# CliMA/LandHydrology.jl

Measured on AMD Instinct MI355X. Metric: column-cell updates/sec (RHS evals), higher is better.
Workload: dtype f64

## Files before the change

landhydrology.jl_amd/csrc/lh_column_ops.hpp:

```cpp
#pragma once
#include "lh_closures.hpp"

namespace lh {

template <typename M>
__device__ __forceinline__ MathTables stage_math_tables(const double* gtab, double* lds) {
    MathTables t;
    t.log_tab = lds;
    t.exp_tab = lds + 2 * LOG_TAB_N;
    if (M::uses_tables) {
        for (int i = threadIdx.x; i < MATH_TAB_DOUBLES; i += blockDim.x) lds[i] = gtab[i];
        __syncthreads();
    }
    return t;
}

template <typename M>
constexpr int implicit_threads() {
    return M::uses_tables ? 512 : 256;
}
template <typename M>
__device__ __forceinline__ M implicit_math(const double* math_tab) {
    __shared__ double s_tab[M::uses_tables ? MATH_TAB_DOUBLES : 2];
    return M(stage_math_tables<M>(math_tab, s_tab));
}
__device__ __forceinline__ int64_t implicit_lane_column() { return int64_t(blockIdx.x) * blockDim.x + threadIdx.x; }

template <typename FT> struct Bits;
template <> struct Bits<double> { using type = unsigned long long; };
template <> struct Bits<float> { using type = unsigned int; };

__device__ __forceinline__ double fmax_ft(double a, double b) { return __builtin_fmax(a, b); }
__device__ __forceinline__ float fmax_ft(float a, float b) { return __builtin_fmaxf(a, b); }
__device__ __forceinline__ double fmin_ft(double a, double b) { return __builtin_fmin(a, b); }
__device__ __forceinline__ float fmin_ft(float a, float b) { return __builtin_fminf(a, b); }

__device__ __forceinline__ float max_nonneg(float a, float b) {
    return __builtin_bit_cast(float, __builtin_elementwise_max(__builtin_bit_cast(int, a), __builtin_bit_cast(int, b)));
}

__device__ __forceinline__ unsigned xcd_block(int xcd_remap) {
    unsigned blk = blockIdx.x;
    if (xcd_remap) {
        const unsigned per = gridDim.x >> 3;
        if (blk < (per << 3)) blk = (blk & 7u) * per + (blk >> 3);
    }
    return blk;
}

template <typename FT>
__device__ __forceinline__ void set_stage_boundary_values(DevParams<FT>& P, const FT* b) {
    P.bc_value[FACE_BOTTOM][COMP_ENERGY] = b[0];
    P.bc_value[FACE_BOTTOM][COMP_HYDROLOGY] = b[1];
    P.bc_value[FACE_TOP][COMP_ENERGY] = b[2];
    P.bc_value[FACE_TOP][COMP_HYDROLOGY] = b[3];
}

template <typename FT, typename M>
__device__ __forceinline__ void flux_scales(const DevParams<FT>& P, const ColC<FT>& c, FT& Ksc, FT& cgw) {
    Ksc = M::is_production ? c.Ksat : FT(1);
    cgw = M::is_production ? c.cgw : P.cg2;
}

template <typename FT, typename M, int MODEL, bool FACTORS, bool NOICE, bool WANT_DT>
__device__ __forceinline__ void cell_closures(const M& mm, const DevParams<FT>& P, const ColC<FT>& c, FT vl, FT ti,
                                              FT re, FT Ta, bool vgf, FT& T, FT& kap, FT& K, FT& psi, FT& E,
                                              float& dpsi, float& ircs) {
    constexpr bool WATER = (MODEL != MODEL_HEAT), HEAT = (MODEL != MODEL_RICHARDS);
    FT rcs = FT(1);
    T = Ta;
    kap = FT(0);
    K = psi = E = FT(0);
    dpsi = ircs = 0.0f;
    if (HEAT) {
        T = temperature_closure<FT, M, NOICE>(mm, P, c, vl, ti, re, rcs);
        kap = kappa_closure<FT, M, NOICE>(mm, P, c, vl, ti);
// ... 62 lines not shown
```

landhydrology.jl_amd/csrc/lh_kernels_impl.hpp:

```cpp
#pragma once
#include "lh_closures.hpp"
#include "lh_column_ops.hpp"
#include "lh_launch.hpp"
#include "lh_dispatch.hpp"
#include "lh_atmos.hpp"
#include <type_traits>

namespace lh {

template <typename FT, int MODEL, bool FACTORS, bool PERCOL, typename M, int MODE>
constexpr bool f32_coupled_vgpr_constants() {
    if (MODEL != MODEL_COUPLED || PERCOL || !M::is_production || !(MODE == 0 || MODE == 4)) return false;
    if (sizeof(FT) == 4 && MODE == 4) return true;
    return !FACTORS;
}

template <typename FT, int MODEL, bool FACTORS, bool PERCOL, typename M, bool NOICE>
constexpr bool heat_vgpr_constants() {
    return sizeof(FT) == 8 && MODEL != MODEL_RICHARDS && M::is_production && !NOICE;
}

template <typename FT, int MODEL, bool FACTORS, bool PERCOL, typename M, int PF, int MODE, bool NOICE = false>
constexpr int rhs_waves_per_simd() {
    constexpr bool F64 = sizeof(FT) == 8, RICHARDS = MODEL == MODEL_RICHARDS;
// ... 45 lines not shown
template <int CPL_, int PF_, bool NT_, bool SEG_>
struct KCfg {
    static constexpr int CPL = CPL_, PF = PF_;
    static constexpr bool NT = NT_, SEG = SEG_;
};

__device__ __forceinline__ void wave_sync() {
    __builtin_amdgcn_fence(__ATOMIC_RELEASE, "wavefront");
    __builtin_amdgcn_wave_barrier();
    __builtin_amdgcn_fence(__ATOMIC_ACQUIRE, "wavefront");
}

template <typename FT>
__device__ __forceinline__ bool finite(FT x) {
    return x - x == FT(0);
}

template <typename M>
constexpr bool noice_exists(bool factors) { return M::is_production && !factors; }
template <typename M, int MODEL>
constexpr bool robust_vg_exists() { return M::uses_tables && MODEL != MODEL_HEAT; }
template <typename CFG>
constexpr bool robust_shape_exists() { return !CFG::NT && !CFG::SEG; }
template <typename M, int MODE>
constexpr bool rhs_mode_exists() { return M::is_production || MODE == 0; }
template <typename FT, int MODEL, bool FACTORS, bool PERCOL, typename CFG, typename M, int MODE, bool NOICE = false, bool VGF = true>
__global__ void __launch_bounds__((rhs_max_threads<M, rhs_waves_per_simd<FT, MODEL, FACTORS, PERCOL, M, CFG::PF, MODE, NOICE>()>()),
                                  (rhs_min_waves<M, rhs_waves_per_simd<FT, MODEL, FACTORS, PERCOL, M, CFG::PF, MODE, NOICE>()>()))
rhs_kernel(const DevParams<FT> P0, const Planes<FT> IN, const Planes<FT> AUX, const Planes<FT> BASE,
           const Planes<FT> OUT, const FT dt_value, const FT* __restrict__ dt_device) {
    constexpr bool WATER = (MODEL != MODEL_HEAT);
    constexpr bool HEAT = (MODEL != MODEL_RICHARDS);
    constexpr bool TEND_MODE = (MODE == 0 || MODE == 4);
    DevParams<FT> P = P0;
    if constexpr (heat_vgpr_constants<FT, MODEL, FACTORS, PERCOL, M, NOICE>() && TEND_MODE && (!FACTORS || PERCOL || MODE == 4)) {
        auto vr = [](FT& x) { asm volatile("" : "+v"(x)); };
        vr(P.rho_c_ds); vr(P.rhocp_l); vr(P.rhocp_i); vr(P.T_ref); vr(P.kappa_sat_unfrozen);
        vr(P.l2_kappa_sat_unfrozen); vr(P.l2_kappa_sat_frozen); vr(P.kersten_exp_unfrozen);
        vr(P.kersten_exp_frozen); vr(P.neg_b_log2e_sc);
        if (MODE != 4) {
            vr(P.rho_i); vr(P.LH_f0); vr(P.inv_dz); vr(P.half_inv_dz);
            if (FACTORS) { vr(P.gamma); vr(P.T_ref_visc); vr(P.Omega); }
        }
    }
    if constexpr (heat_vgpr_constants<FT, MODEL, FACTORS, PERCOL, M, NOICE>() && MODE == 0 && FACTORS && !PERCOL) {
        auto vr = [](FT& x) { asm volatile("" : "+v"(x)); };
        vr(P.rho_c_ds); vr(P.rhocp_l); vr(P.T_ref);
    }
    constexpr int CPL = CFG::CPL, PF = CFG::PF;
    constexpr bool NT = CFG::NT;
    constexpr bool TEND = (MODE == 0 || MODE == 4);
    constexpr bool WANT_DT = (MODE == 4);
    const FT dt = (!TEND && dt_device) ? *dt_device : dt_value;
    __shared__ double s_tab[M::uses_tables ? MATH_TAB_DOUBLES : 2];
    extern __shared__ __align__(16) unsigned char s_dyn[];
    const int n = P.nlev;
    float* s_red = reinterpret_cast<float*>(s_dyn);
    if (WANT_DT) s_red[threadIdx.x] = 0.0f;
    __shared__ unsigned s_waves_done;
    if (WANT_DT && threadIdx.x == 0) s_waves_done = 0u;
    constexpr bool MAY_PROF = (MODEL == MODEL_HEAT) || (MODEL == MODEL_RICHARDS && FACTORS);
    FT* s_pf = reinterpret_cast<FT*>(s_dyn + (WANT_DT ? ((size_t(blockDim.x) * sizeof(float) + 15) & ~size_t(15)) : 0));
    const FT* pf_T = (MAY_PROF && MODEL == MODEL_RICHARDS) ? P.aux_prof[3] : nullptr;
    const FT* pf_vl = (MAY_PROF && MODEL == MODEL_HEAT) ? P.aux_prof[0] : nullptr;
    const FT* pf_ti = (MAY_PROF && MODEL == MODEL_HEAT) ? P.aux_prof[1] : nullptr;
    if constexpr (MAY_PROF) {
        for (int i = threadIdx.x; i < n; i += blockDim.x) {
            if (pf_T) s_pf[i] = pf_T[i];
            if (pf_vl) s_pf[i] = pf_vl[i];
            if (pf_ti) s_pf[n + i] = pf_ti[i];
        }
    }
    const M mm(stage_math_tables<M>(P.math_tab, s_tab));
    if (!M::uses_tables) __syncthreads();

    unsigned blk = blockIdx.x;
    if (P.xcd_remap) {
        const unsigned per = gridDim.x >> 3;
        if (blk < (per << 3)) blk = (blk & 7u) * per + (blk >> 3);
    }
    const int64_t col0 = (int64_t(blk) * blockDim.x + threadIdx.x) * CPL;
    if (col0 >= P.ncols) return;
    const int64_t stride = P.stride;
    constexpr bool SEG = CFG::SEG;
    const int i_lo = SEG ? int(blockIdx.y) * P.seg_len : 0;
    const int i_hi = SEG ? (i_lo + P.seg_len < n ? i_lo + P.seg_len : n) : n;
    const int i_first = (SEG && i_lo > 0) ? i_lo - 1 : 0;
    const int i_end = (SEG && i_hi < n) ? i_hi + 1 : n;
    const unsigned lane_byte = (unsigned)col0 * (unsigned)sizeof(FT);
    const unsigned row_bytes = (unsigned)(stride * (int64_t)sizeof(FT));
    auto rload = [&](const FT* row, FT (&out)[CPL]) { bload<FT, CPL, NT>(row, row_bytes, lane_byte, out); };
    auto rstore = [&](FT* row, const FT (&in)[CPL]) { bstore<FT, CPL, NT>(row, row_bytes, lane_byte, in); };

    const int64_t in0 = SEG ? stride * i_first : 0, out0 = SEG ? stride * i_lo : 0;
    constexpr bool FROM_K1 = (MODE == 5);
    const FT* r_vl = (MODEL == MODEL_HEAT ? AUX.v[0] : (FROM_K1 ? BASE.v[0] : IN.v[0])) + in0;
    const FT* r_ti = NOICE ? nullptr : (MODEL == MODEL_HEAT ? AUX.v[1] : (TEND ? IN.v[1] : BASE.v[1])) + in0;
    const FT* r_re = HEAT ? (FROM_K1 ? BASE.v[2] : IN.v[2]) + in0 : nullptr;
    const FT* r_k1v = (FROM_K1 && WATER) ? IN.v[0] + in0 : nullptr;
    const FT* r_k1e = (FROM_K1 && HEAT) ? IN.v[2] + in0 : nullptr;
    const bool need_Taux = (MODEL == MODEL_RICHARDS) && FACTORS && P.viscosity_kind;
    const FT* r_Ta = need_Taux ? AUX.v[3] + in0 : nullptr;
    const FT* b_vl = ((MODE == 2 || MODE == 3) && WATER) ? BASE.v[0] + out0 : nullptr;
    const FT* b_re = ((MODE == 2 || MODE == 3) && HEAT) ? BASE.v[2] + out0 : nullptr;
    FT* o_vl = WATER ? OUT.v[0] + out0 : nullptr;
    FT* o_re = HEAT ? OUT.v[2] + out0 : nullptr;

    ColC<FT> c[CPL];
    int64_t colj[CPL];
#pragma unroll
    for (int j = 0; j < CPL; ++j) {
        colj[j] = col0 + j < P.ncols ? col0 + j : P.ncols - 1;
        c[j] = make_colc<FT, M>(P, colj[j], PERCOL);
        if (WATER && !NOICE) finish_colc<FT, M>(mm, c[j]);
        if constexpr (M::uses_tables && WATER && !PERCOL && !HEAT) asm volatile("" : "+v"(c[j].e_log2_alpha));
    }
    if constexpr (f32_coupled_vgpr_constants<FT, MODEL, FACTORS, PERCOL, M, MODE>()) {
        auto vr = [](FT& x) { asm volatile("" : "+v"(x)); };
        ColC<FT>& q = c[0];
        vr(q.nu); vr(q.theta_lim); vr(q.theta_r); vr(q.inv_por); vr(q.e_inv_m); vr(q.e_m); vr(q.e_one);
        vr(q.e_inv_n); vr(q.e_log2_alpha); vr(q.Ksat); vr(q.inv_S_s); vr(q.inv_nu); vr(q.k_dry);
        if (!NOICE) vr(q.l2_por);
#pragma unroll
        for (int j = 1; j < CPL; ++j) c[j] = c[0];
    }

    constexpr bool vgf = VGF && M::uses_tables;
    const FT cgT = P.cg2;
    FT cgw[CPL], Ksc[CPL];
#pragma unroll
    for (int j = 0; j < CPL; ++j) flux_scales<FT, M>(P, c[j], Ksc[j], cgw[j]);

    FT vl[CPL], ti[CPL], re[CPL], Ta[CPL];
    FT vl_n[PF][CPL], ti_n[PF][CPL], re_n[PF][CPL], Ta_n[PF][CPL];
    FT kv_n[PF][CPL], ke_n[PF][CPL];
    FT vl_p[CPL], re_p[CPL];
    FT yv[CPL], ye[CPL], yv_p[CPL], ye_p[CPL];
    FT K_p[CPL], psi_p[CPL], T_p[CPL], kap_p[CPL], E_p[CPL];
    FT Fw_lo[CPL], Fe_lo[CPL];
    FT nf_acc = FT(0);
    float dpsi_p[CPL], ircs_p[CPL], DmaxW[CPL], DmaxT[CPL];
    float DmaxWb[CPL];

#pragma unroll
    for (int j = 0; j < CPL; ++j) {
        K_p[j] = psi_p[j] = T_p[j] = kap_p[j] = E_p[j] = Fw_lo[j] = Fe_lo[j] = FT(0);
        vl_p[j] = re_p[j] = FT(0);
        yv[j] = ye[j] = yv_p[j] = ye_p[j] = FT(0);
        vl[j] = ti[j] = re[j] = FT(0);
        Ta[j] = FT(288);
        dpsi_p[j] = DmaxW[j] = DmaxWb[j] = DmaxT[j] = ircs_p[j] = 0.0f;
    }
    int lev_f = i_first;
    auto fetch = [&](int slot) {
        if (MAY_PROF && pf_vl) {
#pragma unroll
            for (int j = 0; j < CPL; ++j) vl_n[slot][j] = s_pf[lev_f];
        } else rload(r_vl, vl_n[slot]);
        if (!NOICE) {
            if (MAY_PROF && pf_ti) {
#pragma unroll
                for (int j = 0; j < CPL; ++j) ti_n[slot][j] = s_pf[n + lev_f];
            } else rload(r_ti, ti_n[slot]);
        }
        if (HEAT) rload(r_re, re_n[slot]);
        if (need_Taux) {
            if (MAY_PROF && pf_T) {
#pragma unroll
                for (int j = 0; j < CPL; ++j) Ta_n[slot][j] = s_pf[lev_f];
            } else rload(r_Ta, Ta_n[slot]);
        }
        ++lev_f;
        if (FROM_K1 && WATER) { rload(r_k1v, kv_n[slot]); r_k1v += stride; }
        if (FROM_K1 && HEAT) { rload(r_k1e, ke_n[slot]); r_k1e += stride; }
        r_vl += stride;
        if (!NOICE) r_ti += stride;
        if (HEAT) r_re += stride;
        if (need_Taux) r_Ta += stride;
    };
#pragma unroll
    for (int k = 0; k < PF; ++k) {
#pragma unroll
        for (int j = 0; j < CPL; ++j) {
            vl_n[k][j] = ti_n[k][j] = re_n[k][j] = kv_n[k][j] = ke_n[k][j] = FT(0);
            Ta_n[k][j] = FT(288);
        }
        if (i_first + k < i_end) fetch(k);
    }

    auto emit = [&](const FT (&Fw_hi)[CPL], const FT (&Fe_hi)[CPL], const FT (&u_vl)[CPL],
                    const FT (&u_re)[CPL], const FT (&y_vl)[CPL], const FT (&y_re)[CPL]) {
        FT dvl[CPL], dre[CPL];
#pragma unroll
        for (int j = 0; j < CPL; ++j) {
            dvl[j] = WATER ? Fw_lo[j] - Fw_hi[j] : FT(0);
            dre[j] = HEAT ? Fe_lo[j] - Fe_hi[j] : FT(0);
            if (CPL == 1 || col0 + j < P.ncols) {
                if (WATER) nf_acc = fma_ft(dvl[j], FT(0), nf_acc);
                if (HEAT) nf_acc = fma_ft(dre[j], FT(0), nf_acc);
            }
        }
        if (TEND) {
            if (WATER) rstore(o_vl, dvl);
            if (HEAT) rstore(o_re, dre);
        } else {
            auto stage = [&](const FT* brow, FT* orow, const FT (&u)[CPL], const FT (&k)[CPL], const FT (&yb)[CPL]) {
                constexpr int STAGE = MODE == 1 ? 0 : (MODE == 3 ? 2 : 1);
                FT b[CPL] = {}, r[CPL];
                if (MODE == 2 || MODE == 3) rload(brow, b);
#pragma unroll
                for (int j = 0; j < CPL; ++j) {
                    if (FROM_K1) b[j] = yb[j];
                    r[j] = ssprk33_stage_value<FT>(STAGE, b[j], u[j], k[j], dt);
                }
                rstore(orow, r);
            };
            if (WATER) stage(b_vl, o_vl, u_vl, dvl, y_vl);
            if (HEAT) stage(b_re, o_re, u_re, dre, y_re);
        }
        if (WATER) {
            o_vl += stride;
            if (MODE == 2 || MODE == 3) b_vl += stride;
        }
        if (HEAT) {
            o_re += stride;
            if (MODE == 2 || MODE == 3) b_re += stride;
        }
    };

    for (int i0 = i_first; i0 < i_end; i0 += PF) {
#pragma unroll
      for (int k = 0; k < PF; ++k) {
        const int i = i0 + k;
        if (PF > 1 && i >= i_end) break;
#pragma unroll
        for (int j = 0; j < CPL; ++j) {
            vl[j] = vl_n[k][j];
            ti[j] = NOICE ? FT(0) : ti_n[k][j];
            re[j] = re_n[k][j];
            Ta[j] = Ta_n[k][j];
// ... 98 lines not shown
                    DmaxT[j] = max_nonneg(DmaxT[j], 4.0f * float(fmax_ft(kap_f, kap_f > FT(0) ? kap_p[j] : FT(0))) * ircs_p[j]);
                }
            }
        }
        emit(Fw, Fe, vl_p, re_p, yv_p, ye_p);
    }
    if (nf_acc != nf_acc) atomicOr(P.status, 1u);
    if (WANT_DT) {
        float dmax = 0.0f;
#pragma unroll
        for (int j = 0; j < CPL; ++j) {
            const float Dj = max_nonneg(max_nonneg(DmaxW[j] * float(Ksc[j]), DmaxWb[j]) * float(FT(1) / (c[j].n * c[j].m)), DmaxT[j]);
            if ((CPL == 1 || col0 + j < P.ncols) && Dj == Dj) dmax = max_nonneg(dmax, Dj);
        }
        float* seg = s_red + (threadIdx.x & ~63u);
        const unsigned l = threadIdx.x & 63u;
        seg[l] = dmax;
#pragma unroll
        for (unsigned off = 32; off > 0; off >>= 1) {
            wave_sync();
            if (l < off) {
                dmax = max_nonneg(dmax, seg[l + off]);
                seg[l] = dmax;
            }
        }
        if (l == 0) {
            const int64_t first_lane = int64_t(blk) * blockDim.x;
            const int64_t lanes_left = (P.ncols + CPL - 1) / CPL - first_lane;
            const unsigned nwaves = blockDim.x >> 6;
            const unsigned nw = lanes_left >= int64_t(blockDim.x) ? nwaves : unsigned((lanes_left + 63) >> 6);
            if (atomicAdd(&s_waves_done, 1u) == nw - 1u) {
                for (unsigned w = 0; w < nwaves; ++w) dmax = max_nonneg(dmax, s_red[w << 6]);
                if (dmax > 0.0f) bound_publish<FT>(P, dt, dmax);
            }
        }
    }
}

constexpr int CS_FACE_WORDS = 8;
template <int MODEL> constexpr int cs_flux_arrays() {
    return MODEL == MODEL_COUPLED ? 2 : 1;
}
static inline int cs_fetch_tiles(int model, bool noice, bool need_Taux) {
    if (model == MODEL_RICHARDS) return 1 + (noice ? 0 : 1) + (need_Taux ? 2 : 0);
    return 3;
}

template <typename FT, int MODEL, bool FACTORS, bool PERCOL, typename M, bool NOICE = false, bool VGF = true>
__global__ void __launch_bounds__(1024)
column_stepper_kernel(const DevParams<FT> P0, const Planes<FT> Y, const Planes<FT> AUX, const FT dt_value,
                      const FT* __restrict__ dt_device, const int64_t nsteps, const FT* __restrict__ bcv) {
    constexpr bool WATER = (MODEL != MODEL_HEAT);
    constexpr bool HEAT = (MODEL != MODEL_RICHARDS);
    __shared__ double s_tab[M::uses_tables ? MATH_TAB_DOUBLES : 2];
    extern __shared__ __align__(16) unsigned char s_dyn[];
    const int n = P0.nlev;
    const int tpc = (n + 63) & ~63;
    const int slot = int(threadIdx.x) / tpc;
    const int cpb = int(blockDim.x) / tpc;
    const FT dt = dt_device ? *dt_device : dt_value;
    constexpr int NARR = cs_exchange_arrays<MODEL>();
    const StepperLds<FT, MODEL> ex(reinterpret_cast<FT*>(s_dyn) + size_t(slot) * NARR * n, n);
    const M mm(stage_math_tables<M>(P0.math_tab, s_tab));
    if (!M::uses_tables) __syncthreads();
    DevParams<FT> P = P0;
    const int i = int(threadIdx.x) - slot * tpc;
    const unsigned blk = xcd_block(P.xcd_remap);
    const int64_t col_raw = int64_t(blk) * cpb + slot;
    const bool cell = i < n && col_raw < P.ncols;
    const int ic = i < n ? i : n - 1;
    const int64_t col = col_raw < P.ncols ? col_raw : P.ncols - 1;
    ColC<FT> c = make_colc<FT, M>(P, col, PERCOL);
    if (WATER && !NOICE) finish_colc<FT, M>(mm, c);
    constexpr bool vgf = VGF && M::uses_tables;
    const FT cgT = P.cg2;
    FT Ksc, cgw;
    flux_scales<FT, M>(P, c, Ksc, cgw);
    const bool need_Taux = (MODEL == MODEL_RICHARDS) && FACTORS && P.viscosity_kind;
    FT* tiles = reinterpret_cast<FT*>(s_dyn);
    const int64_t col_first = int64_t(blk) * cpb;
    const int tile_n = n * cpb;
    auto request = [&](const FT* plane, int k) {
        for (int e = threadIdx.x; e < tile_n; e += blockDim.x) {
            const int lev = e / cpb, cs = e - lev * cpb;
            if (col_first + cs < P.ncols) tiles[k * tile_n + cs * n + lev] = plane[int64_t(lev) * P.stride + col_first + cs];
        }
    };
    auto fetched = [&](int k) -> FT { return (col_raw < P.ncols) ? tiles[k * tile_n + slot * n + ic] : FT(0); };
    const FT* pf_vl = MODEL == MODEL_HEAT ? P.aux_prof[0] : nullptr;
    const FT* pf_ti = MODEL == MODEL_HEAT ? P.aux_prof[1] : nullptr;
    const FT* pf_T = need_Taux ? P.aux_prof[3] : nullptr;
    if (!pf_vl) request(MODEL == MODEL_HEAT ? AUX.v[0] : Y.v[0], 0);
    if (!NOICE && !pf_ti) request(MODEL == MODEL_HEAT ? AUX.v[1] : Y.v[1], 1);
    if (HEAT) request(Y.v[2], 2);
    if (need_Taux && !pf_T) request(AUX.v[3], 3);
    __syncthreads();
    FT y_vl = pf_vl ? pf_vl[ic] : fetched(0);
    const FT ti = NOICE ? FT(0) : (pf_ti ? pf_ti[ic] : fetched(1));
    FT y_re = HEAT ? fetched(2) : FT(0);
    const FT Ta = need_Taux ? (pf_T ? pf_T[ic] : fetched(3)) : FT(288);
    __syncthreads();
    FT nf_acc = FT(0);
    for (int64_t s = 0; s < nsteps; ++s) {
        FT u_vl = y_vl, u_re = y_re;
#pragma unroll 1
        for (int stage = 0; stage < 3; ++stage) {
            if (bcv) set_stage_boundary_values(P, bcv + (s * 3 + stage) * 4);
// ... 41 lines not shown
            const FT dre = HEAT ? Fe_lo - Fe_hi : FT(0);
            if (cell) {
                if (WATER) nf_acc = fma_ft(dvl, FT(0), nf_acc);
                if (HEAT) nf_acc = fma_ft(dre, FT(0), nf_acc);
            }
            if (WATER) u_vl = ssprk33_stage_value<FT>(stage, y_vl, u_vl, dvl, dt);
            if (HEAT) u_re = ssprk33_stage_value<FT>(stage, y_re, u_re, dre, dt);
            __syncthreads();
        }
        y_vl = u_vl;
        y_re = u_re;
    }
    __syncthreads();
    if (i < n) {
        if (WATER) tiles[slot * n + i] = y_vl;
        if (HEAT) tiles[tile_n + slot * n + i] = y_re;
    }
    __syncthreads();
    for (int e = threadIdx.x; e < tile_n; e += blockDim.x) {
        const int lev = e / cpb, cs = e - lev * cpb;
        if (col_first + cs < P.ncols) {
            const int64_t g = int64_t(lev) * P.stride + col_first + cs;
            if (WATER) Y.v[0][g] = tiles[cs * n + lev];
            if (HEAT) Y.v[2][g] = tiles[tile_n + cs * n + lev];
        }
    }
    if (cell && nf_acc != nf_acc) atomicOr(P.status, 1u);
}

template <typename T>
__device__ __forceinline__ T wave_uniform(const T& x) {
    static_assert(sizeof(T) % 4 == 0, "32-bit words");
    uint32_t w[sizeof(T) / 4];
    __builtin_memcpy(w, &x, sizeof(T));
#pragma unroll
    for (size_t k = 0; k < sizeof(T) / 4; ++k) w[k] = __builtin_amdgcn_readfirstlane(w[k]);
    T r;
    __builtin_memcpy(&r, w, sizeof(T));
    return r;
}

template <typename FT, int MODEL, bool FACTORS, bool PERCOL, typename M, int CW, bool NOICE>
constexpr int cs_wave_min_waves() {
    if (!M::uses_tables || MODEL != MODEL_RICHARDS) return 4;
    if (CW == 1) return 6;
    return (NOICE && !FACTORS) ? 6 : 4;
}
template <typename FT, int MODEL, bool FACTORS, bool PERCOL, typename M, int CW, bool NOICE = false, bool VGF = true, bool BOUND = false>
__global__ void __launch_bounds__(1024, (cs_wave_min_waves<FT, MODEL, FACTORS, PERCOL, M, CW, NOICE>()))
column_stepper_wave_kernel(const DevParams<FT> P0, const Planes<FT> Y, const Planes<FT> AUX, const FT dt_value,
                           const FT* __restrict__ dt_device, const int64_t nsteps, const FT* __restrict__ bcv) {
    constexpr bool WATER = (MODEL != MODEL_HEAT);
    constexpr bool HEAT = (MODEL != MODEL_RICHARDS);
    __shared__ double s_tab[M::uses_tables ? MATH_TAB_DOUBLES : 2];
    extern __shared__ __align__(16) unsigned char s_dyn[];
    const int n = P0.nlev;
    const int slot = int(threadIdx.x) >> 6;
    const int l = int(threadIdx.x) & 63;
    const int cpb = int(blockDim.x) >> 6;
    const FT dt = dt_device ? *dt_device : dt_value;
    constexpr int NEX = cs_exchange_arrays<MODEL>();
    constexpr int NARR = NEX + cs_flux_arrays<MODEL>();
    constexpr size_t COLW = size_t(NARR) * 64 + CS_FACE_WORDS;
    const StepperLds<FT, MODEL> ex(reinterpret_cast<FT*>(s_dyn) + size_t(slot) * COLW, 64);
    FT* sFw = ex.K + size_t(NEX) * 64;
    FT* sFe = WATER ? sFw + 64 : sFw;
    FT* sFace = ex.K + size_t(NARR) * 64;
    const M mm(stage_math_tables<M>(P0.math_tab, s_tab));
    if (!M::uses_tables) __syncthreads();
    DevParams<FT> P = P0;
    const unsigned blk = xcd_block(P.xcd_remap);
    const int64_t col_raw = int64_t(blk) * cpb + slot;
    const int64_t col = col_raw < P.ncols ? col_raw : P.ncols - 1;
    ColC<FT> c = make_colc<FT, M>(P, col, PERCOL);
    if (WATER && !NOICE) finish_colc<FT, M>(mm, c);
    if constexpr (PERCOL) c = wave_uniform(c);
    constexpr bool vgf = VGF && M::uses_tables;
    const FT cgT = P.cg2;
    FT Ksc, cgw;
    flux_scales<FT, M>(P, c, Ksc, cgw);
    const bool need_Taux = (MODEL == MODEL_RICHARDS) && FACTORS && P.viscosity_kind;
    FT* tiles = reinterpret_cast<FT*>(s_dyn);
    const int64_t col_first = int64_t(blk) * cpb;
    const int tile_n = n * cpb;
    auto request = [&](const FT* plane, int k) {
        for (int e = threadIdx.x; e < tile_n; e += blockDim.x) {
            const int lev = e / cpb, cs = e - lev * cpb;
            if (col_first + cs < P.ncols) tiles[k * tile_n + cs * n + lev] = plane[int64_t(lev) * P.stride + col_first + cs];
        }
    };
    const FT* pf_vl = MODEL == MODEL_HEAT ? P.aux_prof[0] : nullptr;
    const FT* pf_ti = MODEL == MODEL_HEAT ? P.aux_prof[1] : nullptr;
    const FT* pf_T = need_Taux ? P.aux_prof[3] : nullptr;
    if (!pf_vl) request(MODEL == MODEL_HEAT ? AUX.v[0] : Y.v[0], 0);
    if (!NOICE && !pf_ti) request(MODEL == MODEL_HEAT ? AUX.v[1] : Y.v[1], 1);
    if (HEAT) request(Y.v[2], 2);
    if (need_Taux && !pf_T) request(AUX.v[3], 3);
    __syncthreads();
    FT y_vl[CW], y_re[CW], ti[CW], Ta[CW];
    bool act[CW];
#pragma unroll
    for (int q = 0; q < CW; ++q) {
        const int i = CW * l + q;
        const int ic = i < n ? i : n - 1;
        act[q] = i < n && col_raw < P.ncols;
        const bool have = col_raw < P.ncols;
        y_vl[q] = pf_vl ? pf_vl[ic] : (have ? tiles[slot * n + ic] : FT(0));
// ... 183 lines not shown
            } else {
                const FaceState<FT> fs = face_state<FT, M, MODEL, FACTORS, NOICE>(mm, P, c, face, col, bv, bti, bT, vgf);
                K_f = fs.K;
                kap_f = fs.kap;
            }
            const FT K_c = bK * Ksc;
            DmaxW = max_nonneg(DmaxW, 2.0f * float(bK) * bdpsi);
            DmaxWb = max_nonneg(DmaxWb, 4.0f * float(fmax_ft(K_f, K_f > FT(0) ? K_c : FT(0))) * bdpsi);
            if (HEAT) {
                DmaxT = max_nonneg(DmaxT, 2.0f * float(bkap) * bircs);
                DmaxT = max_nonneg(DmaxT, 4.0f * float(fmax_ft(kap_f, kap_f > FT(0) ? bkap : FT(0))) * bircs);
            }
        };
        if (at_bottom || at_top) boundary_terms(at_bottom ? FACE_BOTTOM : FACE_TOP, at_bottom ? hoist_b : hoist_t, at_bottom ? 0 : qt);
        if (at_bottom && at_top) boundary_terms(FACE_TOP, hoist_t, qt);
#pragma unroll
        for (int off = 32; off > 0; off >>= 1) {
            DmaxW = max_nonneg(DmaxW, __shfl_xor(DmaxW, off, 64));
            DmaxWb = max_nonneg(DmaxWb, __shfl_xor(DmaxWb, off, 64));
            if (HEAT) DmaxT = max_nonneg(DmaxT, __shfl_xor(DmaxT, off, 64));
        }
        if (l == 0 && col_raw < P.ncols) {
            const float Dj = max_nonneg(max_nonneg(DmaxW * float(Ksc), DmaxWb) * float(FT(1) / (c.n * c.m)), DmaxT);
            const float dmax = Dj == Dj ? max_nonneg(0.0f, Dj) : 0.0f;
            if (dmax > 0.0f) bound_publish<FT>(P, courant, dmax);
        }
    }
    __syncthreads();
#pragma unroll
    for (int q = 0; q < CW; ++q) {
        const int i = CW * l + q;
        if (i < n) {
            if (WATER) tiles[slot * n + i] = y_vl[q];
            if (HEAT) tiles[tile_n + slot * n + i] = y_re[q];
        }
    }
    __syncthreads();
    for (int e = threadIdx.x; e < tile_n; e += blockDim.x) {
        const int lev = e / cpb, cs = e - lev * cpb;
        if (col_first + cs < P.ncols) {
            const int64_t g = int64_t(lev) * P.stride + col_first + cs;
            if (WATER) Y.v[0][g] = tiles[cs * n + lev];
            if (HEAT) Y.v[2][g] = tiles[tile_n + cs * n + lev];
        }
    }
    if (col_raw < P.ncols && nf_acc != nf_acc) atomicOr(P.status, 1u);
}

template <typename FT, int MODEL, bool FACTORS, bool PERCOL, typename M>
__global__ void __launch_bounds__(256)
diag_kernel(const DevParams<FT> P, const Planes<FT> IN, const Planes<FT> AUX, const Planes<FT> OUT) {
    constexpr bool WATER = (MODEL != MODEL_HEAT);
    constexpr bool HEAT = (MODEL != MODEL_RICHARDS);
    __shared__ double s_tab[M::uses_tables ? MATH_TAB_DOUBLES : 1];
    const M mm(stage_math_tables<M>(P.math_tab, s_tab));
    const int64_t col = int64_t(blockIdx.x) * blockDim.x + threadIdx.x;
    if (col >= P.ncols) return;
    const FT* p_vl = (MODEL == MODEL_HEAT ? AUX.v[0] : IN.v[0]) + col;
    const FT* p_ti = (MODEL == MODEL_HEAT ? AUX.v[1] : IN.v[1]) + col;
    const bool need_Taux = (MODEL == MODEL_RICHARDS) && FACTORS && P.viscosity_kind;
    ColC<FT> c = make_colc<FT, M>(P, col, PERCOL);
    if (WATER) finish_colc<FT, M>(mm, c);
    const bool vgf = M::uses_tables && P.vg_fast_all != 0;
    for (int i = 0; i < P.nlev; ++i) {
        const int64_t o = int64_t(i) * P.stride;
        FT vl = p_vl[o], ti = p_ti[o];
        FT T = need_Taux ? AUX.v[3][o + col] : FT(288), kap = FT(0), K = FT(0), psi = FT(0);
        if (HEAT) {
            FT rcs;
            T = temperature_closure<FT, M>(mm, P, c, vl, ti, IN.v[2][o + col], rcs);
            kap = kappa_closure<FT, M>(mm, P, c, vl, ti);
        }
        if (WATER) water_closures<FT, M, FACTORS>(mm, P, c, vl, ti, T, K, psi, nullptr, vgf);
        OUT.v[0][o + col] = K;
        OUT.v[1][o + col] = psi;
        OUT.v[2][o + col] = kap;
        OUT.v[3][o + col] = T;
    }
}

template <typename FT, int MODEL, bool FACTORS, bool PERCOL, typename M>
__global__ void __launch_bounds__(256)
boundary_flux_kernel(const DevParams<FT> P, const Planes<FT> IN, const Planes<FT> AUX, const int face, FT* out_e, FT* out_w) {
    constexpr bool WATER = (MODEL != MODEL_HEAT);
    constexpr bool HEAT = (MODEL != MODEL_RICHARDS);
    __shared__ double s_tab[M::uses_tables ? MATH_TAB_DOUBLES : 1];
    const M mm(stage_math_tables<M>(P.math_tab, s_tab));
    const int64_t col = int64_t(blockIdx.x) * blockDim.x + threadIdx.x;
    if (col >= P.ncols) return;
    const int64_t o = int64_t(face == FACE_BOTTOM ? 0 : P.nlev - 1) * P.stride + col;
    ColC<FT> c = make_colc<FT, M>(P, col, PERCOL);
    if (WATER) finish_colc<FT, M>(mm, c);
    const bool vgf = M::uses_tables && P.vg_fast_all != 0;
    const bool need_Taux = (MODEL == MODEL_RICHARDS) && FACTORS && P.viscosity_kind;
    const FT vl = (MODEL == MODEL_HEAT ? AUX.v[0] : IN.v[0])[o];
    const FT ti = (MODEL == MODEL_HEAT ? AUX.v[1] : IN.v[1])[o];
    FT T = need_Taux ? AUX.v[3][o] : FT(288), K = FT(0), psi = FT(0), rcs = FT(1);
    if (HEAT) T = temperature_closure<FT, M>(mm, P, c, vl, ti, IN.v[2][o], rcs);
    constexpr bool RELK = M::is_production;
    if (WATER) {
        water_closures<FT, M, FACTORS, true, false, false, RELK>(mm, P, c, vl, ti, T, K, psi, nullptr, vgf);
        if (RELK) K = K * c.Ksat;
    }
    FT fe, fw;
    boundary_fluxes<FT, M, MODEL, FACTORS, false>(mm, P, c, face, col, vl, ti, T, K, psi, fe, fw, nullptr, nullptr, vgf);
    if (P.bc_kind[face][COMP_ENERGY] == BC_NONE) fe = FT(NAN);
    if (P.bc_kind[face][COMP_HYDROLOGY] == BC_NONE) fw = FT(NAN);
    out_e[col] = fe;
    out_w[col] = fw;
}


template <typename FT, int MODEL, bool PERCOL, typename M>
__global__ void __launch_bounds__(256)
stable_dt_kernel(const DevParams<FT> P, const Planes<FT> IN, const Planes<FT> AUX, const FT courant,
                 typename Bits<FT>::type* out_bits) {
    constexpr bool WATER = (MODEL != MODEL_HEAT);
    constexpr bool HEAT = (MODEL != MODEL_RICHARDS);
    using U = typename Bits<FT>::type;
    __shared__ double s_tab[M::uses_tables ? MATH_TAB_DOUBLES : 1];
    const M mm(stage_math_tables<M>(P.math_tab, s_tab));
    const int64_t col = int64_t(blockIdx.x) * blockDim.x + threadIdx.x;
    FT best = FT(INFINITY);
    if (col < P.ncols) {
        const FT* p_vl = (MODEL == MODEL_HEAT ? AUX.v[0] : IN.v[0]) + col;
        const FT* p_ti = (MODEL == MODEL_HEAT ? AUX.v[1] : IN.v[1]) + col;
        ColC<FT> c = make_colc<FT, M>(P, col, PERCOL);
        if (WATER) finish_colc<FT, M>(mm, c);
        const FT cdz2 = courant * P.dz * P.dz;
        const int n = P.nlev;
        FT K_p = FT(0), dpsi_p = FT(0), kap_p = FT(0), rcs_p = FT(1);
        for (int i = 0; i < n; ++i) {
            const int64_t o = int64_t(i) * P.stride;
            FT vl = p_vl[o], ti = p_ti[o];
            FT K = FT(0), dpsi = FT(0), kap = FT(0), rcs = FT(1);
            FT Tc = FT(288);
            if (MODEL == MODEL_RICHARDS && P.viscosity_kind) Tc = AUX.v[3][o + col];
            if (HEAT) Tc = temperature_closure<FT, M>(mm, P, c, vl, ti, IN.v[2][o + col], rcs);
            if (WATER) {
                FT psi;
                water_closures<FT, M, true>(mm, P, c, vl, ti, Tc, K, psi);
                const FT nu_eff = c.nu - ti;
                const FT vls = !(vl <= c.theta_lim) ? vl : c.theta_lim;
                const FT Se = (vls - c.theta_r) / (nu_eff - c.theta_r);
                const FT u = mm.pow(Se, -c.inv_m) - FT(1);
                if (Se <= FT(1) && u > FT(0))
                    dpsi = fabs(psi) * (u + FT(1)) / (c.n * c.m * u * Se * (nu_eff - c.theta_r));
                else
                    dpsi = FT(1) / c.S_s;
            }
            if (HEAT) kap = kappa_closure<FT, M>(mm, P, c, vl, ti);
            FT D = FT(0);
            if (i == 0 || i == n - 1) {
                D = K * dpsi;
                if (HEAT && kap / rcs > D) D = kap / rcs;
                for (int face = 0; face < 2; ++face) {
                    if ((face == FACE_BOTTOM) != (i == 0) && n > 1) continue;
                    const int kh = P.bc_kind[face][COMP_HYDROLOGY], ke = P.bc_kind[face][COMP_ENERGY];
                    FT vh = P.bc_value[face][COMP_HYDROLOGY];
                    if (P.bc_pc[face][COMP_HYDROLOGY]) vh = P.bc_pc[face][COMP_HYDROLOGY][col];
                    const FT vl_f = (WATER && kh == BC_DIRICHLET) ? vh : vl;
                    FT ve = P.bc_value[face][COMP_ENERGY];
                    if (P.bc_pc[face][COMP_ENERGY]) ve = P.bc_pc[face][COMP_ENERGY][col];
                    const FT T_f = (HEAT && ke == BC_DIRICHLET) ? ve : Tc;
                    if (WATER && kh == BC_DIRICHLET) {
                        FT K_f, psi_f;
                        water_closures<FT, M, true, false>(mm, P, c, vl_f, ti, T_f, K_f, psi_f);
                        FT Db = FT(2) * (K_f > K ? K_f : K) * dpsi;
                        if (Db > D) D = Db;
                    }
                    if (HEAT && ke == BC_DIRICHLET) {
                        FT kf = kappa_closure<FT, M>(mm, P, c, vl_f, ti);
                        FT Db = FT(2) * (kf > kap ? kf : kap) / rcs;
// ... 451 lines not shown
```

landhydrology.jl_amd/csrc/lh_layered.hpp:

```cpp
#pragma once
#include "lh_device.hpp"

namespace lh {

constexpr int LH_LAYERED_MAX_CLASSES = 16;

template <typename FT>
struct LayeredArgs {
    const uint8_t* cls;
    const ColC<FT>* table;
    int32_t ncls;
    int32_t pad_;
};

template <typename FT>
void launch_layered_rhs(const DevParams<FT>& P, const LayeredArgs<FT>& L, const Planes<FT>& in, const Planes<FT>& aux,
                        const Planes<FT>& base, const Planes<FT>& out, FT dt, int mode, bool factors, bool noice,
                        hipStream_t s);
template <typename FT>
void launch_layered_diag(const DevParams<FT>& P, const LayeredArgs<FT>& L, const Planes<FT>& in, const Planes<FT>& aux,
                         const Planes<FT>& out, hipStream_t s);
template <typename FT>
void launch_layered_boundary_fluxes(const DevParams<FT>& P, const LayeredArgs<FT>& L, const Planes<FT>& in,
                                    const Planes<FT>& aux, int face, FT* out_e, FT* out_w, bool factors, hipStream_t s);
// ... 9 lines not shown
namespace lh {


template <typename FT, typename M, bool FINISH>
__device__ __forceinline__ void stage_class_table(const M& mm, const LayeredArgs<FT>& L, ColC<FT>* s_cls) {
    static_assert(sizeof(ColC<FT>) % 4 == 0, "the table is copied in 32-bit words");
    constexpr unsigned W = sizeof(ColC<FT>) / 4;
    const uint32_t* src = reinterpret_cast<const uint32_t*>(L.table);
    uint32_t* dst = reinterpret_cast<uint32_t*>(s_cls);
    const unsigned last = unsigned(L.ncls) - 1u;
    for (unsigned i = threadIdx.x; i < W * LH_LAYERED_MAX_CLASSES; i += blockDim.x) {
        const unsigned e = i / W, w = i - e * W;
        dst[i] = src[(e < last ? e : last) * W + w];
    }
    __syncthreads();
    if (FINISH) {
        if (threadIdx.x < LH_LAYERED_MAX_CLASSES) finish_colc<FT, M>(mm, s_cls[threadIdx.x]);
        __syncthreads();
    }
}

template <int CPL>
__device__ __forceinline__ unsigned cload(const uint8_t* row, unsigned row_bytes, unsigned lane_byte) {
    static_assert(CPL == 1 || CPL == 2, "one or two class bytes per lane");
    __amdgpu_buffer_rsrc_t rs = __builtin_amdgcn_make_buffer_rsrc(const_cast<uint8_t*>(row), 0, row_bytes, 0x00020000);
    if constexpr (CPL == 1) return __builtin_amdgcn_raw_buffer_load_b8(rs, lane_byte, 0, 0);
    else return __builtin_amdgcn_raw_buffer_load_b16(rs, lane_byte, 0, 0);
}
__device__ __forceinline__ unsigned class_of(unsigned packed, int j) {
    return (packed >> (8 * j)) & unsigned(LH_LAYERED_MAX_CLASSES - 1);
}


template <typename M, bool FACTORS, bool NOICE, bool VGF, int MODE>
constexpr bool layered_variant_exists() {
    return M::is_production && (!NOICE || noice_exists<M>(FACTORS)) && (VGF || robust_vg_exists<M, MODEL_RICHARDS>()) &&
           MODE >= 0 && MODE <= 3;
}
template <typename M>
constexpr int layered_threads() { return M::uses_tables ? 512 : 256; }
template <typename FT, typename M, bool FACTORS, bool NOICE>
constexpr int layered_min_waves() {
    if (!M::uses_tables) return 1;
    return (NOICE && !FACTORS) ? 6 : 4;
}

template <typename FT, bool FACTORS, typename M, int MODE, bool NOICE, bool VGF>
__global__ void __launch_bounds__((layered_threads<M>()), (layered_min_waves<FT, M, FACTORS, NOICE>()))
layered_rhs_kernel(const DevParams<FT> P, const LayeredArgs<FT> L, const Planes<FT> IN, const Planes<FT> AUX,
                   const Planes<FT> BASE, const Planes<FT> OUT, const FT dt) {
    using CFG = typename DefaultCfg<FT>::type;
    constexpr int CPL = CFG::CPL, PF = CFG::PF;
    constexpr bool TEND = (MODE == 0);
    __shared__ double s_tab[M::uses_tables ? MATH_TAB_DOUBLES : 2];
    __shared__ ColC<FT> s_cls[LH_LAYERED_MAX_CLASSES];
    const M mm(stage_math_tables<M>(P.math_tab, s_tab));
    stage_class_table<FT, M, !NOICE>(mm, L, s_cls);

    const unsigned blk = xcd_block(P.xcd_remap);
    const int64_t col0 = (int64_t(blk) * blockDim.x + threadIdx.x) * CPL;
    if (col0 >= P.ncols) return;
    const int n = P.nlev;
    const int64_t stride = P.stride;
    const unsigned lane_byte = (unsigned)col0 * (unsigned)sizeof(FT);
    const unsigned row_bytes = (unsigned)(stride * (int64_t)sizeof(FT));
    auto rload = [&](const FT* row, FT (&out)[CPL]) { bload<FT, CPL, false>(row, row_bytes, lane_byte, out); };
    auto rstore = [&](FT* row, const FT (&in)[CPL]) { bstore<FT, CPL, false>(row, row_bytes, lane_byte, in); };

    const FT* r_vl = IN.v[0];
    const FT* r_ti = NOICE ? nullptr : (TEND ? IN.v[1] : BASE.v[1]);
    const bool need_Taux = FACTORS && P.viscosity_kind;
    const FT* r_Ta = need_Taux ? AUX.v[3] : nullptr;
    const uint8_t* r_cls = L.cls;
    const FT* b_vl = (MODE == 2 || MODE == 3) ? BASE.v[0] : nullptr;
    FT* o_vl = OUT.v[0];

    int64_t colj[CPL];
#pragma unroll
    for (int j = 0; j < CPL; ++j) colj[j] = col0 + j < P.ncols ? col0 + j : P.ncols - 1;

    constexpr bool vgf = VGF && M::uses_tables;
    FT vl[CPL], ti[CPL], Ta[CPL];
    FT vl_n[PF][CPL], ti_n[PF][CPL], Ta_n[PF][CPL];
    unsigned kc = 0u, kc_n[PF];
    FT vl_p[CPL];
    FT K_p[CPL], psi_p[CPL];
    FT Fw_lo[CPL];
    FT nf_acc = FT(0);
#pragma unroll
    for (int j = 0; j < CPL; ++j) {
        K_p[j] = psi_p[j] = Fw_lo[j] = vl_p[j] = FT(0);
        vl[j] = ti[j] = FT(0);
        Ta[j] = FT(288);
    }
    auto fetch = [&](int slot) {
        rload(r_vl, vl_n[slot]);
        kc_n[slot] = cload<CPL>(r_cls, (unsigned)stride, (unsigned)col0);
        if (!NOICE) rload(r_ti, ti_n[slot]);
        if (need_Taux) rload(r_Ta, Ta_n[slot]);
        r_vl += stride;
        r_cls += stride;
        if (!NOICE) r_ti += stride;
        if (need_Taux) r_Ta += stride;
    };
#pragma unroll
    for (int k = 0; k < PF; ++k) {
#pragma unroll
// ... 44 lines not shown
        for (int j = 0; j < CPL; ++j) {
            const ColC<FT>& c = s_cls[class_of(kc, j)];
            FT Kr = FT(0);
            psi[j] = FT(0);
            water_closures<FT, M, FACTORS, true, false, NOICE, true, false, true>(mm, P, c, vl[j], ti[j], Ta[j], Kr, psi[j],
                                                                                  nullptr, vgf);
            K[j] = Kr * c.Ksat;
        }
        if (i == 0) {
#pragma unroll
            for (int j = 0; j < CPL; ++j) {
                const ColC<FT>& c = s_cls[class_of(kc, j)];
                FT Fe;
                boundary_fluxes<FT, M, MODEL_RICHARDS, FACTORS, NOICE>(mm, P, c, FACE_BOTTOM, colj[j], vl[j], ti[j], Ta[j],
                                                                       K[j], -psi[j], Fe, Fw_lo[j], nullptr, nullptr, vgf);
                Fw_lo[j] = Fw_lo[j] * P.inv_dz;
            }
        } else {
            FT Fw[CPL];
#pragma unroll
            for (int j = 0; j < CPL; ++j) Fw[j] = -(K_p[j] + K[j]) * (head_difference(psi[j], psi_p[j], P.dz) * P.cg2);
            emit(Fw, vl_p);
#pragma unroll
            for (int j = 0; j < CPL; ++j) Fw_lo[j] = Fw[j];
        }
#pragma unroll
        for (int j = 0; j < CPL; ++j) {
            vl_p[j] = vl[j];
            K_p[j] = K[j];
            psi_p[j] = psi[j];
        }
      }
    }
    {
        FT Fw[CPL];
#pragma unroll
        for (int j = 0; j < CPL; ++j) {
            const ColC<FT>& c = s_cls[class_of(kc, j)];
            FT Fe;
            boundary_fluxes<FT, M, MODEL_RICHARDS, FACTORS, NOICE>(mm, P, c, FACE_TOP, colj[j], vl[j], ti[j], Ta[j], K_p[j],
                                                                   -psi_p[j], Fe, Fw[j], nullptr, nullptr, vgf);
            Fw[j] = Fw[j] * P.inv_dz;
        }
        emit(Fw, vl_p);
    }
    if (nf_acc != nf_acc) atomicOr(P.status, 1u);
}


template <typename FT, typename M>
__global__ void __launch_bounds__(256)
layered_diag_kernel(const DevParams<FT> P, const LayeredArgs<FT> L, const Planes<FT> IN, const Planes<FT> AUX,
                    const Planes<FT> OUT) {
    __shared__ double s_tab[M::uses_tables ? MATH_TAB_DOUBLES : 1];
    __shared__ ColC<FT> s_cls[LH_LAYERED_MAX_CLASSES];
    const M mm(stage_math_tables<M>(P.math_tab, s_tab));
    stage_class_table<FT, M, true>(mm, L, s_cls);
    const int64_t col = int64_t(blockIdx.x) * blockDim.x + threadIdx.x;
    if (col >= P.ncols) return;
    const bool need_Taux = P.viscosity_kind != 0;
    const bool vgf = M::uses_tables && P.vg_fast_all != 0;
    for (int i = 0; i < P.nlev; ++i) {
        const int64_t o = int64_t(i) * P.stride + col;
        const ColC<FT>& c = s_cls[L.cls[o] & (LH_LAYERED_MAX_CLASSES - 1)];
        const FT vl = IN.v[0][o], ti = IN.v[1][o];
        const FT T = need_Taux ? AUX.v[3][o] : FT(288);
        FT K = FT(0), psi = FT(0);
        water_closures<FT, M, true>(mm, P, c, vl, ti, T, K, psi, nullptr, vgf);
        OUT.v[0][o] = K;
        OUT.v[1][o] = psi;
        OUT.v[2][o] = FT(0);
        OUT.v[3][o] = T;
    }
}

template <typename FT, bool FACTORS, typename M>
__global__ void __launch_bounds__(256)
layered_boundary_flux_kernel(const DevParams<FT> P, const LayeredArgs<FT> L, const Planes<FT> IN, const Planes<FT> AUX,
                             const int face, FT* out_e, FT* out_w) {
    __shared__ double s_tab[M::uses_tables ? MATH_TAB_DOUBLES : 1];
    __shared__ ColC<FT> s_cls[LH_LAYERED_MAX_CLASSES];
    const M mm(stage_math_tables<M>(P.math_tab, s_tab));
    stage_class_table<FT, M, true>(mm, L, s_cls);
    const int64_t col = int64_t(blockIdx.x) * blockDim.x + threadIdx.x;
    if (col >= P.ncols) return;
    const int64_t o = int64_t(face == FACE_BOTTOM ? 0 : P.nlev - 1) * P.stride + col;
    const ColC<FT>& c = s_cls[L.cls[o] & (LH_LAYERED_MAX_CLASSES - 1)];
    const bool vgf = M::uses_tables && P.vg_fast_all != 0;
    const bool need_Taux = FACTORS && P.viscosity_kind;
    const FT vl = IN.v[0][o], ti = IN.v[1][o];
    const FT T = need_Taux ? AUX.v[3][o] : FT(288);
    FT K = FT(0), psi = FT(0);
    water_closures<FT, M, FACTORS, true, false, false, true>(mm, P, c, vl, ti, T, K, psi, nullptr, vgf);
    K = K * c.Ksat;
    FT fe, fw;
    boundary_fluxes<FT, M, MODEL_RICHARDS, FACTORS, false>(mm, P, c, face, col, vl, ti, T, K, psi, fe, fw, nullptr, nullptr, vgf);
    const bool bot = (face == FACE_BOTTOM);
    if ((bot ? P.bc_kind[FACE_BOTTOM][COMP_ENERGY] : P.bc_kind[FACE_TOP][COMP_ENERGY]) == BC_NONE) fe = FT(NAN);
    if ((bot ? P.bc_kind[FACE_BOTTOM][COMP_HYDROLOGY] : P.bc_kind[FACE_TOP][COMP_HYDROLOGY]) == BC_NONE) fw = FT(NAN);
    out_e[col] = fe;
    out_w[col] = fw;
}

template <typename FT, typename M>
__global__ void __launch_bounds__(256)
layered_stable_dt_kernel(const DevParams<FT> P, const LayeredArgs<FT> L, const Planes<FT> IN, const Planes<FT> AUX,
                         const FT courant, typename Bits<FT>::type* out_bits) {
    using U = typename Bits<FT>::type;
    __shared__ double s_tab[M::uses_tables ? MATH_TAB_DOUBLES : 1];
    __shared__ ColC<FT> s_cls[LH_LAYERED_MAX_CLASSES];
    const M mm(stage_math_tables<M>(P.math_tab, s_tab));
    stage_class_table<FT, M, true>(mm, L, s_cls);
    const int64_t col = int64_t(blockIdx.x) * blockDim.x + threadIdx.x;
    FT best = FT(INFINITY);
    if (col < P.ncols) {
        const FT cdz2 = courant * P.dz * P.dz;
        const int n = P.nlev;
        FT K_p = FT(0), dpsi_p = FT(0);
        for (int i = 0; i < n; ++i) {
            const int64_t o = int64_t(i) * P.stride + col;
            const ColC<FT>& c = s_cls[L.cls[o] & (LH_LAYERED_MAX_CLASSES - 1)];
            const FT vl = IN.v[0][o], ti = IN.v[1][o];
            const FT Tc = P.viscosity_kind ? AUX.v[3][o] : FT(288);
            FT K = FT(0), dpsi = FT(0), psi;
            water_closures<FT, M, true>(mm, P, c, vl, ti, Tc, K, psi);
            const FT nu_eff = c.nu - ti;
            const FT vls = !(vl <= c.theta_lim) ? vl : c.theta_lim;
            const FT Se = (vls - c.theta_r) / (nu_eff - c.theta_r);
            const FT u = mm.pow(Se, -c.inv_m) - FT(1);
            if (Se <= FT(1) && u > FT(0))
                dpsi = fabs(psi) * (u + FT(1)) / (c.n * c.m * u * Se * (nu_eff - c.theta_r));
            else
                dpsi = FT(1) / c.S_s;
            FT D = FT(0);
            if (i == 0 || i == n - 1) {
                D = K * dpsi;
                for (int face = 0; face < 2; ++face) {
                    if ((face == FACE_BOTTOM) != (i == 0) && n > 1) continue;
                    if (P.bc_kind[face][COMP_HYDROLOGY] != BC_DIRICHLET) continue;
                    FT vh = P.bc_value[face][COMP_HYDROLOGY];
                    if (P.bc_pc[face][COMP_HYDROLOGY]) vh = P.bc_pc[face][COMP_HYDROLOGY][col];
                    FT K_f, psi_f;
                    water_closures<FT, M, true, false>(mm, P, c, vh, ti, Tc, K_f, psi_f);
                    const FT Db = FT(2) * (K_f > K ? K_f : K) * dpsi;
                    if (Db > D) D = Db;
                }
            }
            if (i > 0) {
                const FT Dw = (K_p + K) * FT(0.5) * (dpsi_p > dpsi ? dpsi_p : dpsi);
                if (Dw > D) D = Dw;
            }
            if (D > FT(0)) {
                const FT dtc = cdz2 / D;
                if (dtc < best) best = dtc;
            }
            K_p = K;
            dpsi_p = dpsi;
        }
    }
#pragma unroll
    for (int off = 32; off > 0; off >>= 1) {
        const FT other = __shfl_down(best, off, 64);
// ... 67 lines not shown
```

Baseline: 285.1 billion.

## Stage math tables via async global-to-LDS loads overlapped with prologue prefetch

Replaces the per-thread copy of the log/exp lookup tables into LDS with 16-byte global_load_lds DMA transfers. The work is split into an issue step and a commit step (a waitcnt plus a barrier). In the main RHS kernel, the commit and finish_colc are deferred until after the first level prefetches are issued, so table staging overlaps with column loads. Out-of-range lanes now stay alive until after the barrier and load from a safe offset. This adds complexity, including a hardcoded waitcnt encoding and a requirement for 16-byte LDS alignment, and it holds more registers live across the prologue.

```diff
diff --git a/landhydrology.jl_amd/csrc/lh_column_ops.hpp b/landhydrology.jl_amd/csrc/lh_column_ops.hpp
--- a/landhydrology.jl_amd/csrc/lh_column_ops.hpp
+++ b/landhydrology.jl_amd/csrc/lh_column_ops.hpp
@@ -3,15 +3,32 @@
 
 namespace lh {
 
+constexpr unsigned MATH_TAB_PIECES = MATH_TAB_DOUBLES / 2;
+static_assert(MATH_TAB_DOUBLES % 2 == 0 && MATH_TAB_PIECES % 64 == 0, "16-byte pieces, whole waves");
 template <typename M>
-__device__ __forceinline__ MathTables stage_math_tables(const double* gtab, double* lds) {
+__device__ __forceinline__ MathTables stage_math_tables_issue(const double* gtab, double* lds) {
     MathTables t;
     t.log_tab = lds;
     t.exp_tab = lds + 2 * LOG_TAB_N;
     if (M::uses_tables) {
-        for (int i = threadIdx.x; i < MATH_TAB_DOUBLES; i += blockDim.x) lds[i] = gtab[i];
+        typedef __attribute__((address_space(1))) const void* gptr_t;
+        typedef __attribute__((address_space(3))) void* lptr_t;
+        for (unsigned i = threadIdx.x; i < MATH_TAB_PIECES; i += blockDim.x)
+            __builtin_amdgcn_global_load_lds((gptr_t)(gtab + 2 * i), (lptr_t)(lds + 2 * i), 16, 0, 0);
+    }
+    return t;
+}
+template <typename M>
+__device__ __forceinline__ void stage_math_tables_commit() {
+    if (M::uses_tables) {
+        __builtin_amdgcn_s_waitcnt(0x0F70);
         __syncthreads();
     }
+}
+template <typename M>
+__device__ __forceinline__ MathTables stage_math_tables(const double* gtab, double* lds) {
+    const MathTables t = stage_math_tables_issue<M>(gtab, lds);
+    stage_math_tables_commit<M>();
     return t;
 }
 
@@ -21,7 +38,7 @@
 }
 template <typename M>
 __device__ __forceinline__ M implicit_math(const double* math_tab) {
-    __shared__ double s_tab[M::uses_tables ? MATH_TAB_DOUBLES : 2];
+    __shared__ __align__(16) double s_tab[M::uses_tables ? MATH_TAB_DOUBLES : 2];
     return M(stage_math_tables<M>(math_tab, s_tab));
 }
 __device__ __forceinline__ int64_t implicit_lane_column() { return int64_t(blockIdx.x) * blockDim.x + threadIdx.x; }
diff --git a/landhydrology.jl_amd/csrc/lh_kernels_impl.hpp b/landhydrology.jl_amd/csrc/lh_kernels_impl.hpp
--- a/landhydrology.jl_amd/csrc/lh_kernels_impl.hpp
+++ b/landhydrology.jl_amd/csrc/lh_kernels_impl.hpp
@@ -121,7 +121,7 @@
     constexpr bool TEND = (MODE == 0 || MODE == 4);
     constexpr bool WANT_DT = (MODE == 4);
     const FT dt = (!TEND && dt_device) ? *dt_device : dt_value;
-    __shared__ double s_tab[M::uses_tables ? MATH_TAB_DOUBLES : 2];
+    __shared__ __align__(16) double s_tab[M::uses_tables ? MATH_TAB_DOUBLES : 2];
     extern __shared__ __align__(16) unsigned char s_dyn[];
     const int n = P.nlev;
     float* s_red = reinterpret_cast<float*>(s_dyn);
@@ -140,8 +140,12 @@
             if (pf_ti) s_pf[n + i] = pf_ti[i];
         }
     }
-    const M mm(stage_math_tables<M>(P.math_tab, s_tab));
-    if (!M::uses_tables) __syncthreads();
+    constexpr bool EARLY = M::uses_tables && !MAY_PROF;
+    const M mm(stage_math_tables_issue<M>(P.math_tab, s_tab));
+    if constexpr (!EARLY) {
+        stage_math_tables_commit<M>();
+        if (!M::uses_tables) __syncthreads();
+    }
 
     unsigned blk = blockIdx.x;
     if (P.xcd_remap) {
@@ -149,15 +153,15 @@
         if (blk < (per << 3)) blk = (blk & 7u) * per + (blk >> 3);
     }
     const int64_t col0 = (int64_t(blk) * blockDim.x + threadIdx.x) * CPL;
-    if (col0 >= P.ncols) return;
+    if (!EARLY && col0 >= P.ncols) return;
     const int64_t stride = P.stride;
     constexpr bool SEG = CFG::SEG;
     const int i_lo = SEG ? int(blockIdx.y) * P.seg_len : 0;
     const int i_hi = SEG ? (i_lo + P.seg_len < n ? i_lo + P.seg_len : n) : n;
     const int i_first = (SEG && i_lo > 0) ? i_lo - 1 : 0;
     const int i_end = (SEG && i_hi < n) ? i_hi + 1 : n;
-    const unsigned lane_byte = (unsigned)col0 * (unsigned)sizeof(FT);
     const unsigned row_bytes = (unsigned)(stride * (int64_t)sizeof(FT));
+    const unsigned lane_byte = (EARLY && col0 >= P.ncols) ? row_bytes : (unsigned)col0 * (unsigned)sizeof(FT);
     auto rload = [&](const FT* row, FT (&out)[CPL]) { bload<FT, CPL, NT>(row, row_bytes, lane_byte, out); };
     auto rstore = [&](FT* row, const FT (&in)[CPL]) { bstore<FT, CPL, NT>(row, row_bytes, lane_byte, in); };
 
@@ -181,7 +185,9 @@
     for (int j = 0; j < CPL; ++j) {
         colj[j] = col0 + j < P.ncols ? col0 + j : P.ncols - 1;
         c[j] = make_colc<FT, M>(P, colj[j], PERCOL);
-        if (WATER && !NOICE) finish_colc<FT, M>(mm, c[j]);
+        if constexpr (!EARLY) {
+            if (WATER && !NOICE) finish_colc<FT, M>(mm, c[j]);
+        }
         if constexpr (M::uses_tables && WATER && !PERCOL && !HEAT) asm volatile("" : "+v"(c[j].e_log2_alpha));
     }
     if constexpr (f32_coupled_vgpr_constants<FT, MODEL, FACTORS, PERCOL, M, MODE>()) {
@@ -255,6 +261,14 @@
             Ta_n[k][j] = FT(288);
         }
         if (i_first + k < i_end) fetch(k);
+    }
+    if constexpr (EARLY) {
+        stage_math_tables_commit<M>();
+        if (col0 >= P.ncols) return;
+#pragma unroll
+        for (int j = 0; j < CPL; ++j) {
+            if (WATER && !NOICE) finish_colc<FT, M>(mm, c[j]);
+        }
     }
 
     auto emit = [&](const FT (&Fw_hi)[CPL], const FT (&Fe_hi)[CPL], const FT (&u_vl)[CPL],
@@ -459,7 +473,7 @@
                       const FT* __restrict__ dt_device, const int64_t nsteps, const FT* __restrict__ bcv) {
     constexpr bool WATER = (MODEL != MODEL_HEAT);
     constexpr bool HEAT = (MODEL != MODEL_RICHARDS);
-    __shared__ double s_tab[M::uses_tables ? MATH_TAB_DOUBLES : 2];
+    __shared__ __align__(16) double s_tab[M::uses_tables ? MATH_TAB_DOUBLES : 2];
     extern __shared__ __align__(16) unsigned char s_dyn[];
     const int n = P0.nlev;
     const int tpc = (n + 63) & ~63;
@@ -607,7 +621,7 @@
                            const FT* __restrict__ dt_device, const int64_t nsteps, const FT* __restrict__ bcv) {
     constexpr bool WATER = (MODEL != MODEL_HEAT);
     constexpr bool HEAT = (MODEL != MODEL_RICHARDS);
-    __shared__ double s_tab[M::uses_tables ? MATH_TAB_DOUBLES : 2];
+    __shared__ __align__(16) double s_tab[M::uses_tables ? MATH_TAB_DOUBLES : 2];
     extern __shared__ __align__(16) unsigned char s_dyn[];
     const int n = P0.nlev;
     const int slot = int(threadIdx.x) >> 6;
@@ -897,7 +911,7 @@
 diag_kernel(const DevParams<FT> P, const Planes<FT> IN, const Planes<FT> AUX, const Planes<FT> OUT) {
     constexpr bool WATER = (MODEL != MODEL_HEAT);
     constexpr bool HEAT = (MODEL != MODEL_RICHARDS);
-    __shared__ double s_tab[M::uses_tables ? MATH_TAB_DOUBLES : 1];
+    __shared__ __align__(16) double s_tab[M::uses_tables ? MATH_TAB_DOUBLES : 1];
     const M mm(stage_math_tables<M>(P.math_tab, s_tab));
     const int64_t col = int64_t(blockIdx.x) * blockDim.x + threadIdx.x;
     if (col >= P.ncols) return;
@@ -929,7 +943,7 @@
 boundary_flux_kernel(const DevParams<FT> P, const Planes<FT> IN, const Planes<FT> AUX, const int face, FT* out_e, FT* out_w) {
     constexpr bool WATER = (MODEL != MODEL_HEAT);
     constexpr bool HEAT = (MODEL != MODEL_RICHARDS);
-    __shared__ double s_tab[M::uses_tables ? MATH_TAB_DOUBLES : 1];
+    __shared__ __align__(16) double s_tab[M::uses_tables ? MATH_TAB_DOUBLES : 1];
     const M mm(stage_math_tables<M>(P.math_tab, s_tab));
     const int64_t col = int64_t(blockIdx.x) * blockDim.x + threadIdx.x;
     if (col >= P.ncols) return;
@@ -963,7 +977,7 @@
     constexpr bool WATER = (MODEL != MODEL_HEAT);
     constexpr bool HEAT = (MODEL != MODEL_RICHARDS);
     using U = typename Bits<FT>::type;
-    __shared__ double s_tab[M::uses_tables ? MATH_TAB_DOUBLES : 1];
+    __shared__ __align__(16) double s_tab[M::uses_tables ? MATH_TAB_DOUBLES : 1];
     const M mm(stage_math_tables<M>(P.math_tab, s_tab));
     const int64_t col = int64_t(blockIdx.x) * blockDim.x + threadIdx.x;
     FT best = FT(INFINITY);
diff --git a/landhydrology.jl_amd/csrc/lh_layered.hpp b/landhydrology.jl_amd/csrc/lh_layered.hpp
--- a/landhydrology.jl_amd/csrc/lh_layered.hpp
+++ b/landhydrology.jl_amd/csrc/lh_layered.hpp
@@ -85,7 +85,7 @@
     using CFG = typename DefaultCfg<FT>::type;
     constexpr int CPL = CFG::CPL, PF = CFG::PF;
     constexpr bool TEND = (MODE == 0);
-    __shared__ double s_tab[M::uses_tables ? MATH_TAB_DOUBLES : 2];
+    __shared__ __align__(16) double s_tab[M::uses_tables ? MATH_TAB_DOUBLES : 2];
     __shared__ ColC<FT> s_cls[LH_LAYERED_MAX_CLASSES];
     const M mm(stage_math_tables<M>(P.math_tab, s_tab));
     stage_class_table<FT, M, !NOICE>(mm, L, s_cls);
@@ -236,7 +236,7 @@
 __global__ void __launch_bounds__(256)
 layered_diag_kernel(const DevParams<FT> P, const LayeredArgs<FT> L, const Planes<FT> IN, const Planes<FT> AUX,
                     const Planes<FT> OUT) {
-    __shared__ double s_tab[M::uses_tables ? MATH_TAB_DOUBLES : 1];
+    __shared__ __align__(16) double s_tab[M::uses_tables ? MATH_TAB_DOUBLES : 1];
     __shared__ ColC<FT> s_cls[LH_LAYERED_MAX_CLASSES];
     const M mm(stage_math_tables<M>(P.math_tab, s_tab));
     stage_class_table<FT, M, true>(mm, L, s_cls);
@@ -262,7 +262,7 @@
 __global__ void __launch_bounds__(256)
 layered_boundary_flux_kernel(const DevParams<FT> P, const LayeredArgs<FT> L, const Planes<FT> IN, const Planes<FT> AUX,
                              const int face, FT* out_e, FT* out_w) {
-    __shared__ double s_tab[M::uses_tables ? MATH_TAB_DOUBLES : 1];
+    __shared__ __align__(16) double s_tab[M::uses_tables ? MATH_TAB_DOUBLES : 1];
     __shared__ ColC<FT> s_cls[LH_LAYERED_MAX_CLASSES];
     const M mm(stage_math_tables<M>(P.math_tab, s_tab));
     stage_class_table<FT, M, true>(mm, L, s_cls);
@@ -291,7 +291,7 @@
 layered_stable_dt_kernel(const DevParams<FT> P, const LayeredArgs<FT> L, const Planes<FT> IN, const Planes<FT> AUX,
                          const FT courant, typename Bits<FT>::type* out_bits) {
     using U = typename Bits<FT>::type;
-    __shared__ double s_tab[M::uses_tables ? MATH_TAB_DOUBLES : 1];
+    __shared__ __align__(16) double s_tab[M::uses_tables ? MATH_TAB_DOUBLES : 1];
     __shared__ ColC<FT> s_cls[LH_LAYERED_MAX_CLASSES];
     const M mm(stage_math_tables<M>(P.math_tab, s_tab));
     stage_class_table<FT, M, true>(mm, L, s_cls);
```

Measured after the change: 287.5 billion, median of 6. About the same (+0.8%).
